# relgukxilef/GAN-Class-Transfer2

Hardware: AMD Instinct MI355X
Metric: images/sec (train step) 3x128x128 bs=64/GPU (higher is better)
Workload: dtype bf16; 1 GPU; BASELINE config 3: Trainer step, 3x128x128, bs 64/GPU, octaves 6, pixel_size 128, max_size 512, bf16 operands / fp32 accumulate, Keras Adam + WarmUp; global_batch=64, parallelism=dp1

## Files before the change

gan-class-transfer2_amd/csrc/halo_mfma.hip:

```cpp
#include "gct2_common.h"
#include <algorithm>
#include <type_traits>

namespace {

constexpr unsigned OOB = 0x80000000u;
typedef __attribute__((address_space(3))) void lds_void_t;

__device__ __forceinline__ __amdgpu_buffer_rsrc_t make_rsrc(const void* base) {
  return __builtin_amdgcn_make_buffer_rsrc(const_cast<void*>(base), 0, (int)OOB, 0x00020000);
}
__device__ __forceinline__ void dma16(__amdgpu_buffer_rsrc_t rsrc, char* lds_piece, unsigned voff) {
  __builtin_amdgcn_raw_ptr_buffer_load_lds(rsrc, (lds_void_t*)lds_piece, 16, (int)voff, 0, 0, 0);
}
__device__ __forceinline__ void dma16s(__amdgpu_buffer_rsrc_t rsrc, char* lds_piece, unsigned voff, unsigned soff) {
  __builtin_amdgcn_raw_ptr_buffer_load_lds(rsrc, (lds_void_t*)lds_piece, 16, (int)voff, (int)soff, 0, 0);
}
__device__ __forceinline__ int halo_swz(int row) { return (((row >> 1) & 1) << 2) | (((row >> 2) & 1) << 1); }
__device__ __forceinline__ int w_row(int i, int q) { return 32 * (i >> 1) + 8 * (q >> 2) + 4 * (i & 1) + (q & 3); }
__device__ __forceinline__ int w_swz(int n) { return (((n >> 3) & 1) << 1) | (((n >> 1) & 1) << 2); }

constexpr int HP = 18;
constexpr int HPIECES = 41;
constexpr int HALO_BYTES = HPIECES * 1024;
constexpr int WB_BYTES = 4 * 64 * 128;

#ifdef GCT2_STAMP
__device__ __forceinline__ unsigned long long stamp() {
  unsigned long long t;
  __builtin_amdgcn_sched_barrier(0);
  asm volatile("s_memrealtime %0\n\ts_waitcnt lgkmcnt(0)" : "=s"(t)::"memory");
  __builtin_amdgcn_sched_barrier(0);
  return t;
}
#define STAMP(k) st[k] = stamp()
#else
#define STAMP(k)
#endif
template <typename T, int EPI>
__global__ __launch_bounds__(512, 2) void halo_convT_kernel(TapGemmParams p) {
#ifdef GCT2_STAMP
  unsigned long long st[6];
  STAMP(0);
#endif
  constexpr int HEAD_CT_OFF = 2 * HALO_BYTES + 2 * WB_BYTES, HEAD_CT_BYTES = 14 * 1024;
  __shared__ __attribute__((aligned(16))) char lds_all[2 * HALO_BYTES + 2 * WB_BYTES + (EPI == EPI_HEAD ? HEAD_CT_BYTES : 0)];
  char* const halo0 = lds_all;
  char* const halo1 = lds_all + HALO_BYTES;
  char* const wb0 = lds_all + 2 * HALO_BYTES;
  char* const wb1 = lds_all + 2 * HALO_BYTES + WB_BYTES;

  GCT2_CLOCK_DECL;
  const int tid = threadIdx.x, lane = tid & 63;
  const int wave = __builtin_amdgcn_readfirstlane(tid >> 6);
  const int phase = wave >> 1, mhalf = wave & 1;
  const int ph = phase >> 1, pw = phase & 1;
  const int g = lane >> 4, q = lane & 15;
  const int Hs = p.Hs, Ws = p.Ws, K = p.K, N = p.N;
  const int tx_n = Ws >> 4, ty_n = Hs >> 4;
  int m_tile, n_tile;
  if (!xcd_tile((int)blockIdx.x, p.m_tiles, p.n_tiles, p.xcd_chunk, m_tile, n_tile)) return;
  const int tx = m_tile % tx_n, tq = m_tile / tx_n, ty = tq % ty_n, b = tq / ty_n;
  const int sh0 = ty * 16, sw0 = tx * 16, n0 = n_tile * 64;
  const __amdgpu_buffer_rsrc_t rs_x = make_rsrc(p.x), rs_w = make_rsrc(p.w);
  const int ldx2 = p.ldx * 2;

  unsigned h_voff[6];
  int h_lchunk[6];
#pragma unroll
  for (int i = 0; i < 6; i++) {
    const int pi = wave + 8 * i;
    const int row = 8 * pi + (lane >> 3);
    const int hy = row / HP, hx = row - hy * HP;
    const int lchunk = (lane & 7) ^ halo_swz(hx);
    h_lchunk[i] = lchunk;
    h_voff[i] = OOB;
    if (pi < HPIECES && row < HP * HP) {
      const int y = sh0 - 1 + hy, x = sw0 - 1 + hx;
      if ((unsigned)y < (unsigned)Hs && (unsigned)x < (unsigned)Ws) h_voff[i] = (unsigned)(((b * Hs + y) * Ws + x) * ldx2 + lchunk * 16);
    }
  }
  const int w_n = 8 * wave + (lane >> 3);
  const int w_lchunk = (lane & 7) ^ w_swz(w_n);
  const unsigned w_voff = (n0 + w_n) < N ? (unsigned)(((n0 + w_n) * K + w_lchunk * 8) * 2) : OOB;
  const unsigned NK2 = (unsigned)(N * K * 2);

  const int nk = (K + 63) / 64;
  const int nround = 4 * nk;

  auto issue_halo = [&](int kc, char* hbuf) {
    const int c0 = kc * 64;
#pragma unroll
    for (int i = 0; i < 6; i++) {
      const int pi = wave + 8 * i;
      if (pi < HPIECES)
        dma16s(rs_x, hbuf + pi * 1024, (c0 + h_lchunk[i] * 8) < K ? h_voff[i] : OOB, (unsigned)(c0 * 2));
    }
  };
  auto issue_w = [&](int round, char* wbuf) {
    const int kc = round >> 2, a = (round >> 1) & 1, c = round & 1;
    const int c0 = kc * 64;
    const unsigned voff = (c0 + w_lchunk * 8) < K ? w_voff : OOB;
#pragma unroll
    for (int i = 0; i < 4; i++) {
      const int tap16 = (1 - (i >> 1) + 2 * a) * 4 + (1 - (i & 1) + 2 * c);
      dma16s(rs_w, wbuf + i * 8192 + wave * 1024, voff, (unsigned)tap16 * NK2 + (unsigned)(c0 * 2));
    }
  };
// ... 87 lines not shown
  }
  asm volatile("s_waitcnt vmcnt(0)" ::: "memory");
  __syncthreads();
#define GCT2_LEAN_ROUND(FAST, R, IDX, HCUR, HNEXT, WCUR, WNEXT)                              \
  {                                                                                          \
    lean_round(std::integral_constant<bool, FAST>{}, (R), IDX, HCUR, HNEXT, WCUR, WNEXT);    \
    asm volatile("s_waitcnt vmcnt(0)" ::: "memory");                                         \
    __syncthreads();                                                                         \
    if (!FAST && (R) + 1 >= nround) break;                                                   \
  }
#define GCT2_LEAN_TRIP(FAST)                                                                 \
  GCT2_LEAN_ROUND(FAST, r + 0, 0, 0, HALO_BYTES, 0, WB_BYTES)                                \
  GCT2_LEAN_ROUND(FAST, r + 1, 1, 0, HALO_BYTES, WB_BYTES, 0)                                \
  GCT2_LEAN_ROUND(FAST, r + 2, 2, 0, HALO_BYTES, 0, WB_BYTES)                                \
  GCT2_LEAN_ROUND(FAST, r + 3, 3, 0, HALO_BYTES, WB_BYTES, 0)                                \
  GCT2_LEAN_ROUND(FAST, r + 4, 4, HALO_BYTES, 0, 0, WB_BYTES)                                \
  GCT2_LEAN_ROUND(FAST, r + 5, 5, HALO_BYTES, 0, WB_BYTES, 0)                                \
  GCT2_LEAN_ROUND(FAST, r + 6, 6, HALO_BYTES, 0, 0, WB_BYTES)                                \
  GCT2_LEAN_ROUND(FAST, r + 7, 7, HALO_BYTES, 0, WB_BYTES, 0)
  {
    int r = 0;
    for (; r + 8 < kfull4; r += 8) { GCT2_LEAN_TRIP(true) }
    for (; r < nround; r += 8) { GCT2_LEAN_TRIP(false) }
  }
#undef GCT2_LEAN_TRIP
#undef GCT2_LEAN_ROUND
#ifdef GCT2_STAMP
  GCT2_CLOCK_END(p.clock ? p.stamps : nullptr, 8, wave, lane);
#endif

  T* __restrict__ yout = reinterpret_cast<T*>(p.y);
  const T* __restrict__ actp = reinterpret_cast<const T*>(p.act);
  int elane = lane;
  asm volatile("" : "+v"(elane));
  const int eq = elane & 15, eg = elane >> 4;
  if constexpr (EPI == EPI_HEAD) {
    STAMP(1);
    const HeadFuse& hd = p.head;
    const int Cout = hd.Cout;
    constexpr int YP_WAVE = 64 * 128;
    constexpr int CT_OFF = HEAD_CT_OFF;
    constexpr int DT_OFF = 8 * YP_WAVE;
    constexpr int DT_WAVE = 2 * 3 * 64 * 2;
    constexpr int PC_OFF = DT_OFF + 8 * DT_WAVE;
    constexpr int LB_OFF = PC_OFF + 64;
    static_assert(LB_OFF + 256 <= HEAD_CT_OFF, "epilogue LDS map");
    auto fsw = [](int k) { return ((k >> 1) & 1) | (((k >> 3) & 1) << 1); };
    auto term_bits = head_term_bits;
    const T* __restrict__ x2 = reinterpret_cast<const T*>(hd.x2);
    const int nimg = (x2 != nullptr) ? min(hd.Cin - 64, 3) : 0;
    if (tid < 16) {
      const int c = tid >> 2, o = tid & 3;
      float v = 0.f;
      if (o < Cout) v = c < 3 ? (c < nimg ? hd.w[(64 + c) * Cout + o] : 0.f) : (hd.b ? hd.b[o] : 0.f);
      reinterpret_cast<float*>(lds_all + PC_OFF)[tid] = v;
    }
    if (tid >= 64 && tid < 128) reinterpret_cast<float*>(lds_all + LB_OFF)[tid - 64] = p.bias ? p.bias[tid - 64] : 0.f;
    __syncthreads();
    STAMP(2);
    const float gscale = (hd.loss_scale ? *hd.loss_scale : 1.f) * 2.0f / hd.count;
    float bacc[16];
    float wimg[3][3], dbd[3] = {0.f, 0.f, 0.f}, lacc = 0.f;
#pragma unroll
    for (int c = 0; c < 16; c++) bacc[c] = 0.f;
#pragma unroll
    for (int c = 0; c < 3; c++) wimg[c][0] = wimg[c][1] = wimg[c][2] = 0.f;
    f32x4_t accW[4];
#pragma unroll
    for (int f = 0; f < 4; f++) accW[f] = f32x4_t{0.f, 0.f, 0.f, 0.f};
    char* const ypark = lds_all + wave * YP_WAVE;
    char* const dtab = lds_all + DT_OFF + wave * DT_WAVE;
    const size_t pix0 = ((size_t)b * (2 * Hs) + 2 * (sh0 + mhalf * 8) + ph) * (2 * Ws) + 2 * (sw0 + eq) + pw;
    const size_t pix_step = (size_t)4 * Ws;
    auto row_pix = [&](int j) { return pix0 + (size_t)j * pix_step; };
    float tg_n[3] = {0.f, 0.f, 0.f};
    u32x2_t im_n = {0u, 0u};
    auto prefetch = [&](int j) {
      const size_t px = row_pix(j);
#pragma unroll
      for (int o = 0; o < 3; o++) tg_n[o] = o < Cout ? hd.target[px * Cout + o] : 0.f;
      if (nimg > 0) im_n = *reinterpret_cast<const u32x2_t*>(x2 + px * hd.ldx2);
    };
    prefetch(0);
#pragma unroll
    for (int j = 0; j < 8; j++) {
      int ct = CT_OFF + elane * 16;
      asm volatile("" : "+v"(ct));
      const size_t opix = row_pix(j);
      const float tg[3] = {tg_n[0], tg_n[1], tg_n[2]};
      const u32x2_t v2 = im_n;
      if (j < 7) prefetch(j + 1);
      const int krow = (j & 3) * 16 + eq;
      u32x4_t yv[2];
#pragma unroll
      for (int ip = 0; ip < 2; ip++) {
        const f32x4_t b0 = *reinterpret_cast<const f32x4_t*>(lds_all + LB_OFF + (32 * ip + 8 * eg) * 4);
        const f32x4_t b1 = *reinterpret_cast<const f32x4_t*>(lds_all + LB_OFF + (32 * ip + 8 * eg + 4) * 4);
        const f32x4_t v0 = acc[2 * ip][j] + b0, v1 = acc[2 * ip + 1][j] + b1;
        yv[ip] = u32x4_t{pack2<T>(fmaxf(v0[0], 0.f), fmaxf(v0[1], 0.f)), pack2<T>(fmaxf(v0[2], 0.f), fmaxf(v0[3], 0.f)),
                         pack2<T>(fmaxf(v1[0], 0.f), fmaxf(v1[1], 0.f)), pack2<T>(fmaxf(v1[2], 0.f), fmaxf(v1[3], 0.f))};
        *reinterpret_cast<u32x4_t*>(ypark + krow * 128 + (((2 * ip + (eg >> 1)) ^ fsw(krow)) << 5) + (eg & 1) * 16) = yv[ip];
      }
      f32x4_t accP = {0.f, 0.f, 0.f, 0.f};
#pragma unroll
      for (int t = 0; t < 3; t++)
#pragma unroll
        for (int kk = 0; kk < 2; kk++) accP = mfma16<T>(lds_read128(lds_all, ct + (t * 2 + kk) * 1024), yv[kk], accP);
      float dsc[3] = {0.f, 0.f, 0.f};
      if (eg == 0) {
        const float im[3] = {unpack_lo<T>(v2[0]), unpack_hi<T>(v2[0]), unpack_lo<T>(v2[1])};
        f32x4_t pc[4];
#pragma unroll
        for (int c = 0; c < 4; c++) pc[c] = *reinterpret_cast<const f32x4_t*>(lds_all + PC_OFF + 16 * c);
#pragma unroll
        for (int o = 0; o < 3; o++) {
          float s = accP[o];
#pragma unroll
          for (int c = 0; c < 3; c++) s = fmaf(im[c], pc[c][o], s);
          const float pr = keras_f16_point<T>(s + pc[3][o]);
          const float d = o < Cout ? pr - tg[o] : 0.f;
          if (o < Cout) {
            if (hd.pred) hd.pred[opix * Cout + o] = pr;
            lacc = fmaf(d, d, lacc);
          }
          dsc[o] = keras_f16_point<T>(d * gscale);
          dbd[o] += dsc[o];
#pragma unroll
          for (int c = 0; c < 3; c++) wimg[c][o] = fmaf(im[c], dsc[o], wimg[c][o]);
        }
      }
      u32x4_t dB[2];
#pragma unroll
      for (int t = 0; t < 2; t++) {
        const uint32_t d0 = term_bits(dsc[0], t), d1 = term_bits(dsc[1], t), d2 = term_bits(dsc[2], t);
        dB[t] = u32x4_t{d0 | (d1 << 16), d2, 0u, 0u};
        if (eg == 0) {
          uint16_t* dt = reinterpret_cast<uint16_t*>(dtab) + (t * 3) * 64 + krow;
          dt[0] = (uint16_t)d0; dt[64] = (uint16_t)d1; dt[128] = (uint16_t)d2;
        }
      }
#pragma unroll
      for (int ip = 0; ip < 2; ip++) {
        f32x4_t gq[2];
#pragma unroll
        for (int h = 0; h < 2; h++) {
          const int f = 2 * ip + h;
          const u32x4_t wh = lds_read128(lds_all, ct + (6 + f * 2) * 1024), wl = lds_read128(lds_all, ct + (7 + f * 2) * 1024);
          f32x4_t a = mfma16<T>(wh, dB[0], f32x4_t{0.f, 0.f, 0.f, 0.f});
          a = mfma16<T>(wh, dB[1], a);
          gq[h] = mfma16<T>(wl, dB[0], a);
        }
        apply_relu_bits8(relu_bits8<T>(yv[ip]), gq[0], gq[1]);
#pragma unroll
        for (int k = 0; k < 4; k++) { bacc[8 * ip + k] += gq[0][k]; bacc[8 * ip + 4 + k] += gq[1][k]; }
        const u32x4_t o = {pack2<T>(gq[0][0], gq[0][1]), pack2<T>(gq[0][2], gq[0][3]), pack2<T>(gq[1][0], gq[1][1]), pack2<T>(gq[1][2], gq[1][3])};
        *reinterpret_cast<u32x4_t*>(yout + opix * p.ldy + 32 * ip + 8 * eg) = o;
      }
      if ((j & 3) == 3) {
        asm volatile("" ::: "memory");
        const int wo = elane & 15, kg = elane >> 4;
        const int g4 = elane >> 4, q4 = (elane >> 2) & 3, pq = elane & 3;
#pragma unroll
        for (int ks = 0; ks < 2; ks++) {
          u32x4_t da[2];
#pragma unroll
          for (int t = 0; t < 2; t++) {
            da[t] = lds_read128(dtab, ((t * 3 + (wo < 3 ? wo : 0)) * 64 + 32 * ks + 8 * kg) * 2);
            if (wo >= 3) da[t] = u32x4_t{0u, 0u, 0u, 0u};
          }
          const int k0 = 32 * ks + 8 * g4 + q4;
#pragma unroll
          for (int f = 0; f < 4; f++) {
            const int o0 = k0 * 128 + ((f ^ fsw(k0)) << 5) + pq * 8;
            const s16x4_t lo = __builtin_amdgcn_ds_read_tr16_b64_v4i16((lds_s16x4_t*)(ypark + o0));
            const s16x4_t hi = __builtin_amdgcn_ds_read_tr16_b64_v4i16((lds_s16x4_t*)(ypark + o0 + 4 * 128));
            const u32x2_t l2 = __builtin_bit_cast(u32x2_t, lo), h2 = __builtin_bit_cast(u32x2_t, hi);
            const u32x4_t yb = {l2[0], l2[1], h2[0], h2[1]};
            accW[f] = mfma16<T>(da[0], yb, accW[f]);
            accW[f] = mfma16<T>(da[1], yb, accW[f]);
          }
        }
        asm volatile("" ::: "memory");
      }
    }
    STAMP(3);
    __syncthreads();
    STAMP(4);
    float* red = reinterpret_cast<float*>(lds_all);
    for (int i = tid; i < 8 * HEAD_ROW; i += 512) red[i] = 0.f;
    __syncthreads();
    float* rw = red + wave * HEAD_ROW;
    if (eg == 0) {
#pragma unroll
      for (int f = 0; f < 4; f++)
#pragma unroll
        for (int o = 0; o < 3; o++)
          if (o < Cout) rw[(16 * f + eq) * Cout + o] = accW[f][o];
    }
#pragma unroll
    for (int c = 0; c < 16; c++) {
      const float tb = row16_sum(bacc[c]);
      if (eq == 0) rw[224 + 32 * (c >> 3) + 8 * eg + (c & 7)] = tb;
    }
#pragma unroll
    for (int o = 0; o < 3; o++) {
      const float td = row16_sum(dbd[o]);
      if (elane == 0 && o < Cout) rw[216 + o] = td;
#pragma unroll
      for (int c = 0; c < 3; c++) {
        const float tw = row16_sum(wimg[c][o]);
        if (elane == 0 && o < Cout && c < nimg) rw[(64 + c) * Cout + o] = tw;
      }
    }
    {
      const float t = row16_sum(lacc);
      if (elane == 0) rw[219] = t;
    }
    __syncthreads();
    if (tid < HEAD_ROW) {
      float t = red[tid];
#pragma unroll
      for (int k = 1; k < 8; k++) t += red[k * HEAD_ROW + tid];
      hd.part[(size_t)m_tile * HEAD_ROW + tid] = t;
    }
#ifdef GCT2_STAMP
    STAMP(5);
    if (p.stamps && (tid & 63) == 0) {
      unsigned long long* o = p.stamps + ((size_t)m_tile * 8 + wave) * 8;
      for (int k = 0; k < 6; k++) o[k] = st[k];
    }
    GCT2_CLOCK_EXIT(p.clock ? p.stamps : nullptr, 8, wave, lane);
#endif
    return;
  }
  f32x4_t bsum[4];
#pragma unroll
  for (int i = 0; i < 4; i++) bsum[i] = f32x4_t{0.f, 0.f, 0.f, 0.f};
  auto out_pixel = [&](int j) {
    const int sh = sh0 + mhalf * 8 + j, sw = sw0 + eq;
    return ((size_t)b * (2 * Hs) + 2 * sh + ph) * (2 * Ws) + 2 * sw + pw;
  };
  u32x4_t mk[2] = {u32x4_t{0u, 0u, 0u, 0u}, u32x4_t{0u, 0u, 0u, 0u}};
  auto load_masks = [&](int j, u32x4_t* dst) {
    if (EPI == EPI_MASK && actp) {
      const size_t opix = out_pixel(j);
#pragma unroll
      for (int ip = 0; ip < 2; ip++) {
        const int n = n0 + 32 * ip + 8 * eg;
        if (n >= N) continue;
        if (p.bits) dst[ip][0] = p.bits[opix * p.ldbits + (n >> 3)];
        else dst[ip] = *reinterpret_cast<const u32x4_t*>(actp + opix * p.ldact + n);
      }
    }
  };
  load_masks(0, mk);
#pragma unroll
  for (int j = 0; j < 8; j++) {
    u32x4_t mkn[2] = {u32x4_t{0u, 0u, 0u, 0u}, u32x4_t{0u, 0u, 0u, 0u}};
    if (j + 1 < 8) load_masks(j + 1, mkn);
    const size_t opix = out_pixel(j);
    unsigned wbits[2] = {0u, 0u};
#pragma unroll
    for (int ip = 0; ip < 2; ip++) {
      const int n = n0 + 32 * ip + 8 * eg;
      if (n >= N) continue;
      f32x4_t v0 = acc[2 * ip][j], v1 = acc[2 * ip + 1][j];
      if (EPI == EPI_BIAS_ACT) {
        if (p.bias) {
          v0 += *reinterpret_cast<const f32x4_t*>(p.bias + n);
          v1 += *reinterpret_cast<const f32x4_t*>(p.bias + n + 4);
        }
        if (p.relu) {
#pragma unroll
          for (int r = 0; r < 4; r++) { v0[r] = fmaxf(v0[r], 0.f); v1[r] = fmaxf(v1[r], 0.f); }
        }
      } else {
        if (actp && p.bits) apply_relu_bits8(mk[ip][0], v0, v1);
        else if (actp) {
          const u32x4_t a4 = mk[ip];
#pragma unroll
          for (int h = 0; h < 2; h++) {
            if (!(unpack_lo<T>(a4[h]) > 0.f)) v0[2 * h] = 0.f;
            if (!(unpack_hi<T>(a4[h]) > 0.f)) v0[2 * h + 1] = 0.f;
            if (!(unpack_lo<T>(a4[2 + h]) > 0.f)) v1[2 * h] = 0.f;
            if (!(unpack_hi<T>(a4[2 + h]) > 0.f)) v1[2 * h + 1] = 0.f;
          }
        }
        bsum[2 * ip] += v0;
        bsum[2 * ip + 1] += v1;
        if (p.accumulate) {
          const u32x4_t o4 = *reinterpret_cast<const u32x4_t*>(yout + opix * p.ldy + n);
#pragma unroll
          for (int h = 0; h < 2; h++) {
            v0[2 * h] += unpack_lo<T>(o4[h]); v0[2 * h + 1] += unpack_hi<T>(o4[h]);
            v1[2 * h] += unpack_lo<T>(o4[2 + h]); v1[2 * h + 1] += unpack_hi<T>(o4[2 + h]);
          }
        }
      }
      const u32x4_t o = {pack2<T>(v0[0], v0[1]), pack2<T>(v0[2], v0[3]), pack2<T>(v1[0], v1[1]), pack2<T>(v1[2], v1[3])};
      *reinterpret_cast<u32x4_t*>(yout + opix * p.ldy + n) = o;
      if (EPI == EPI_BIAS_ACT && p.bits && !p.bits_words) p.bits[opix * p.ldbits + (n >> 3)] = (unsigned char)relu_bits8<T>(o);
      if (EPI == EPI_BIAS_ACT && p.bits_words) wbits[ip] = relu_bits8<T>(o) << (8 * eg);
    }
    if (EPI == EPI_BIAS_ACT && p.bits_words) {
#pragma unroll
      for (int ip = 0; ip < 2; ip++) {
        const unsigned wd = rows4_or(wbits[ip]);
        if (eg == 0 && n0 + 32 * ip < N) *reinterpret_cast<unsigned*>(p.bits + opix * p.ldbits + ((n0 + 32 * ip) >> 3)) = wd;
      }
    }
    mk[0] = mkn[0]; mk[1] = mkn[1];
    __builtin_amdgcn_sched_barrier(0);
  }
  if (EPI == EPI_MASK && (p.db || p.db2)) {
    float* red = reinterpret_cast<float*>(wb0);
#pragma unroll
    for (int i = 0; i < 4; i++) {
#pragma unroll
      for (int r = 0; r < 4; r++) {
        float t = bsum[i][r];
        t = row16_sum(t);
        const int c = 32 * (i >> 1) + 8 * eg + 4 * (i & 1) + r;
        if (eq == 0) {
          if (p.dbws) red[wave * 64 + c] = t;
          else if (n0 + c < N) {
            float* qd = (n0 + c) < p.db_split ? (p.db ? p.db + n0 + c : nullptr) : (p.db2 ? p.db2 + (n0 + c - p.db_split) : nullptr);
            if (qd) atomicAdd(qd, t);
          }
        }
      }
    }
    if (p.dbws) {
      __syncthreads();
      if (tid < 64 && n0 + tid < N) {
        float t = red[tid];
#pragma unroll
        for (int k = 1; k < 8; k++) t += red[k * 64 + tid];
        p.dbws[(size_t)m_tile * N + n0 + tid] = t;
      }
    }
  }
#ifdef GCT2_STAMP
  GCT2_CLOCK_EXIT(p.clock ? p.stamps : nullptr, 8, wave, lane);
#endif
}

}

bool halo_convT_wanted(const gct2_ctx& c, int epi, const TapGemmParams& p) {
  const int g_halo_mode = c.halo_mode;
  if (g_halo_mode == 1) return false;
  if ((p.Hs & 15) || (p.Ws & 15)) return false;
  if ((uintptr_t)p.y % 16 || p.ldy % 8 || (p.act && ((uintptr_t)p.act % 16 || p.ldact % 8))) return false;
  if (g_halo_mode == 2) return true;
  const int tiles = p.B * (p.Hs >> 4) * (p.Ws >> 4) * ((p.N + 63) / 64);
  return p.N <= 256 && tiles >= 256;
}

bool halo_head_supported(const gct2_ctx& c, int dtype, const TapGemmParams& p) {
  if (dtype != GCT2_BF16 && dtype != GCT2_F16) return false;
  if (p.N != 64 || (p.Hs & 15) || (p.Ws & 15) || p.K % 8 || p.ldx % 8) return false;
  if ((uintptr_t)p.y % 16 || p.ldy % 8 || (uintptr_t)p.x % 16 || (uintptr_t)p.w % 16) return false;
  const size_t src_bytes = (size_t)p.B * p.Hs * p.Ws * p.ldx * 2, lane_max = 7 * 16 + 16, scalar_max = (size_t)p.K * 2;
  const size_t w_bytes = (size_t)16 * p.K * p.N * 2;
  if (src_bytes + lane_max + scalar_max >= 0x7ff00000u || w_bytes >= 0x7ff00000u) return false;
  const size_t rows = (size_t)p.B * (p.Hs >> 4) * (p.Ws >> 4);
  return c.ws && c.ws_bytes >= rows * HEAD_ROW * sizeof(float);
}
int halo_head(gct2_ctx& c, int dtype, TapGemmParams p, float* dw, float* db, float* loss, float* db_up, int accumulate,
              hipStream_t s) {
  p.m_tiles = p.B * (p.Hs >> 4) * (p.Ws >> 4);
  p.n_tiles = 1;
  p.xcd_chunk = (p.m_tiles + 7) / 8;
  p.ksplit = 1;
// ... 56 lines not shown
```

gan-class-transfer2_amd/csrc/tapgemm_mfma.hip:

```cpp
#include "gct2_common.h"
#include <algorithm>


namespace {

constexpr int BK = 64;
constexpr unsigned OOB = 0x80000000u;
#define VMCNT_ONLY(n) ((((n) & 0xF) | 0x70 | 0xF00 | ((((n) >> 4) & 3) << 14)))
typedef __attribute__((address_space(3))) void lds_void_t;

__device__ __forceinline__ __amdgpu_buffer_rsrc_t make_rsrc(const void* base) {
  return __builtin_amdgcn_make_buffer_rsrc(const_cast<void*>(base), 0, (int)OOB, 0x00020000);
}
__device__ __forceinline__ void dma16(__amdgpu_buffer_rsrc_t rsrc, char* lds_piece, unsigned voff) {
  __builtin_amdgcn_raw_ptr_buffer_load_lds(rsrc, (lds_void_t*)lds_piece, 16, (int)voff, 0, 0, 0);
}
__device__ __forceinline__ void dma16s(__amdgpu_buffer_rsrc_t rsrc, char* lds_piece, unsigned voff, unsigned soff) {
  __builtin_amdgcn_raw_ptr_buffer_load_lds(rsrc, (lds_void_t*)lds_piece, 16, (int)voff, (int)soff, 0, 0);
}

__device__ __forceinline__ float* db_target(const TapGemmParams& p, int n) {
  return n < p.db_split ? (p.db ? p.db + n : nullptr) : (p.db2 ? p.db2 + (n - p.db_split) : nullptr);
}
__device__ __forceinline__ bool db_adds(const TapGemmParams& p, int n) { return (p.db_acc >> (n < p.db_split ? 0 : 1)) & 1; }

#ifdef GCT2_STAMP
__device__ __forceinline__ unsigned long long tg_stamp() {
  unsigned long long t;
  __builtin_amdgcn_sched_barrier(0);
  asm volatile("s_memrealtime %0\n\ts_waitcnt lgkmcnt(0)" : "=s"(t)::"memory");
  __builtin_amdgcn_sched_barrier(0);
  return t;
}
#define TG_STAMP(k) st[k] = tg_stamp()
#else
#define TG_STAMP(k)
#endif
template <typename T, int FORM, int BM, int BN, int EPI, int NBUF>
__global__ __launch_bounds__((BM / 64) * (BN / 64) * 64, NBUF == 1 ? 4 : 2) void tapgemm_kernel(TapGemmParams p) {
  constexpr int WM = 64;
  constexpr int NWV = (BM / WM) * (BN / 64);
  constexpr int MF = WM / 16;
  static_assert(NBUF == 1 || NBUF == 2, "one or two LDS buffers");
  static_assert(NWV == 4 || NWV == 8, "4 or 8 waves");
  constexpr bool S1 = (FORM == FORM_S1 || FORM == FORM_S1T);
  constexpr bool WT = (FORM == FORM_CONV || FORM == FORM_S1);
  static_assert(!WT || BN % 128 == 0, "T images are 128 columns wide");
  constexpr int WAVES_N = BN / 64;
  constexpr int BKS = BK;
  constexpr int NA = BM / 8 / NWV;
  constexpr int NW = (WT ? 16 * (BN / 128) : BN / 8) / NWV;
  constexpr int A_BYTES = BM * 128;
  constexpr int W_BYTES = WT ? 64 * 256 * (BN / 128) : BN * 128;
  constexpr int NTAPS = (FORM == FORM_CONV) ? 16 : 4;

  __shared__ __attribute__((aligned(16))) char lds0[A_BYTES + W_BYTES];
  __shared__ __attribute__((aligned(16))) char lds1[NBUF >= 2 ? A_BYTES + W_BYTES : 16];

#ifdef GCT2_STAMP
  unsigned long long st[5];
  unsigned long long* stamp_out = p.stamps;
  TG_STAMP(0);
#endif
  GCT2_CLOCK_DECL;
  const int tid = threadIdx.x, lane = tid & 63;
  const int wave = __builtin_amdgcn_readfirstlane(tid >> 6);
  const int wn = wave % WAVES_N, wm = wave / WAVES_N;
  const int Hs = p.Hs, Ws = p.Ws, K = p.K, N = p.N;
  const int M = p.B * Hs * Ws;
  constexpr int PH = (FORM == FORM_CONVT) ? 4 : 1;
  const int inner = p.n_tiles * PH, per_slice = 8 * p.xcd_chunk * inner;
  int kslice, m_tile, in;
  if (p.wstat) {
    const int xcd = (int)blockIdx.x & 7, j = (int)blockIdx.x >> 3;
    const int slice = (j / p.m_tiles) * 8 + xcd;
    if (slice >= inner * p.ksplit) return;
    m_tile = j % p.m_tiles;
    kslice = slice / inner;
    in = slice - kslice * inner;
  } else {
    kslice = (int)blockIdx.x / per_slice;
    if (!xcd_tile((int)blockIdx.x - kslice * per_slice, p.m_tiles, inner, p.xcd_chunk, m_tile, in)) return;
  }
  const int phase = in % PH, n_tile = in / PH;
  const int m0 = m_tile * BM, n0 = n_tile * BN;
  const int ph = phase >> 1, pw = phase & 1;
  const int Hsrc = (FORM == FORM_CONV) ? 2 * Hs : Hs, Wsrc = (FORM == FORM_CONV) ? 2 * Ws : Ws;
  const __amdgpu_buffer_rsrc_t rs_x = make_rsrc(p.x), rs_w = make_rsrc(p.w);
  const int ldx2 = p.ldx * 2;
// ... 138 lines not shown
    const char* w_img = a_img + A_BYTES;
#pragma unroll
    for (int kk = 0; kk < 2; kk++) {
      u32x4_t wf[4], af[MF];
#pragma unroll
      for (int i = 0; i < 4; i++)
        wf[i] = WT ? timg_frag(w_img + (wn >> 1) * (64 * 256), (wn & 1) * 64 + i * 16, kk, lane)
                                    : nimg_frag(w_img, wn * 64 + i * 16, kk, lane);
#pragma unroll
      for (int j = 0; j < MF; j++) af[j] = nimg_frag(a_img, wm * WM + j * 16, kk, lane);
#pragma unroll
      for (int i = 0; i < 4; i++)
#pragma unroll
        for (int j = 0; j < MF; j++) acc[i][j] = mfma16<T>(wf[i], af[j], acc[i][j]);
    }
  };
  const bool live = p.ksplit > 0;
  TG_STAMP(1);
  GCT2_CLOCK_BEGIN;
  if constexpr (NBUF == 1) {
    for (int it = it_lo; it < it_hi; it++) {
      issue(it, lds0);
      asm volatile("s_waitcnt vmcnt(0)" ::: "memory");
      __syncthreads();
      if (live) compute(lds0);
      __syncthreads();
    }
  } else if constexpr (NBUF == 2) {
    if (it_lo < it_hi) issue(it_lo, lds0);
    asm volatile("s_waitcnt vmcnt(0)" ::: "memory");
    __syncthreads();
    for (int it = it_lo; it < it_hi; it += 2) {
      if (it + 1 < it_hi) issue(it + 1, lds1);
      if (live) compute(lds0);
      asm volatile("s_waitcnt vmcnt(0)" ::: "memory");
      __syncthreads();
      if (it + 1 >= it_hi) break;
      if (it + 2 < it_hi) issue(it + 2, lds0);
      if (live) compute(lds1);
      asm volatile("s_waitcnt vmcnt(0)" ::: "memory");
      __syncthreads();
    }
  }

#ifdef GCT2_STAMP
  GCT2_CLOCK_END(p.clock ? p.stamps : nullptr, NWV, wave, lane);
#endif
  TG_STAMP(2);
  T* __restrict__ yout = reinterpret_cast<T*>(p.y);
  const T* __restrict__ actp = reinterpret_cast<const T*>(p.act);
  int elane = lane;
  asm volatile("" : "+v"(elane));
  f32x4_t bsum[4];
#pragma unroll
  for (int i = 0; i < 4; i++) bsum[i] = f32x4_t{0.f, 0.f, 0.f, 0.f};
  const bool wide = p.wide && p.ksplit == 1;
  if (wide) {
    const int eg = elane >> 4;
    const int nlane = wn * 64 + 16 * (eg & 1) + 4 * (eg & ~1);
    auto out_pixel = [&](int j, size_t& opix) -> bool {
      const int m = m0 + wm * WM + j * 16 + (elane & 15);
      if (m >= M) return false;
      if (FORM != FORM_CONVT) opix = (size_t)m;
      else {
        int sw, sh, b;
        decode_pixel(m, Hs, Ws, p.hs_shift, p.ws_shift, sw, sh, b);
        opix = ((size_t)b * (2 * Hs) + 2 * sh + ph) * (2 * Ws) + 2 * sw + pw;
      }
      return true;
    };
    u32x4_t mk[2] = {u32x4_t{0u, 0u, 0u, 0u}, u32x4_t{0u, 0u, 0u, 0u}};
    auto load_masks = [&](int j, u32x4_t* dst) {
      size_t opix;
      if (EPI == EPI_MASK && actp && out_pixel(j, opix)) {
#pragma unroll
        for (int ip = 0; ip < 2; ip++) {
          const int n = n0 + nlane + 32 * ip;
          if (n >= N) continue;
          if (p.bits) dst[ip][0] = p.bits[opix * p.ldbits + (n >> 3)];
          else dst[ip] = *reinterpret_cast<const u32x4_t*>(actp + opix * p.ldact + n);
        }
      }
    };
    load_masks(0, mk);
#pragma unroll
    for (int j = 0; j < MF; j++) {
      u32x4_t mkn[2] = {u32x4_t{0u, 0u, 0u, 0u}, u32x4_t{0u, 0u, 0u, 0u}};
      if (j + 1 < MF) load_masks(j + 1, mkn);
      f32x4_t v0[2], v1[2];
#pragma unroll
      for (int ip = 0; ip < 2; ip++) {
#pragma unroll
        for (int r = 0; r < 4; r++) {
          float xa = acc[2 * ip][j][r], xb = acc[2 * ip + 1][j][r];
          asm volatile("v_permlane16_swap_b32 %0, %1" : "+v"(xa), "+v"(xb));
          v0[ip][r] = xa;
          v1[ip][r] = xb;
        }
      }
      size_t opix;
      const bool row_ok = out_pixel(j, opix);
      unsigned wbits[2] = {0u, 0u};
#pragma unroll
      for (int ip = 0; ip < 2; ip++) {
        const int n = n0 + nlane + 32 * ip;
        if (!row_ok || n >= N) continue;
        f32x4_t a = v0[ip], c = v1[ip];
        if (EPI == EPI_BIAS_ACT) {
          if (p.bias) {
            a += *reinterpret_cast<const f32x4_t*>(p.bias + n);
            c += *reinterpret_cast<const f32x4_t*>(p.bias + n + 4);
          }
          if (p.relu) {
#pragma unroll
            for (int r = 0; r < 4; r++) { a[r] = fmaxf(a[r], 0.f); c[r] = fmaxf(c[r], 0.f); }
          }
        } else {
          if (actp && p.bits) apply_relu_bits8(mk[ip][0], a, c);
          else if (actp) {
            const u32x4_t a4 = mk[ip];
#pragma unroll
            for (int h = 0; h < 2; h++) {
              if (!(unpack_lo<T>(a4[h]) > 0.f)) a[2 * h] = 0.f;
              if (!(unpack_hi<T>(a4[h]) > 0.f)) a[2 * h + 1] = 0.f;
              if (!(unpack_lo<T>(a4[2 + h]) > 0.f)) c[2 * h] = 0.f;
              if (!(unpack_hi<T>(a4[2 + h]) > 0.f)) c[2 * h + 1] = 0.f;
            }
          }
          bsum[2 * ip] += a;
          bsum[2 * ip + 1] += c;
          if (p.accumulate) {
            const u32x4_t o4 = *reinterpret_cast<const u32x4_t*>(yout + opix * p.ldy + n);
#pragma unroll
            for (int h = 0; h < 2; h++) {
              a[2 * h] += unpack_lo<T>(o4[h]); a[2 * h + 1] += unpack_hi<T>(o4[h]);
              c[2 * h] += unpack_lo<T>(o4[2 + h]); c[2 * h + 1] += unpack_hi<T>(o4[2 + h]);
            }
          }
        }
        const u32x4_t o = {pack2<T>(a[0], a[1]), pack2<T>(a[2], a[3]), pack2<T>(c[0], c[1]), pack2<T>(c[2], c[3])};
        *reinterpret_cast<u32x4_t*>(yout + opix * p.ldy + n) = o;
        if (EPI == EPI_BIAS_ACT && p.bits && !p.bits_words) p.bits[opix * p.ldbits + (n >> 3)] = (unsigned char)relu_bits8<T>(o);
        if (EPI == EPI_BIAS_ACT && p.bits_words) wbits[ip] = relu_bits8<T>(o) << (((n >> 3) & 3) * 8);
      }
      if (EPI == EPI_BIAS_ACT && p.bits_words) {
#pragma unroll
        for (int ip = 0; ip < 2; ip++) {
          const unsigned wd = rows4_or(wbits[ip]);
          const int n32 = n0 + wn * 64 + 32 * ip;
          if (eg == 0 && row_ok && n32 < N) *reinterpret_cast<unsigned*>(p.bits + opix * p.ldbits + (n32 >> 3)) = wd;
        }
      }
      mk[0] = mkn[0]; mk[1] = mkn[1];
      __builtin_amdgcn_sched_barrier(0);
    }
  } else {
#pragma unroll
  for (int j = 0; j < MF; j++) {
    const int m = m0 + wm * WM + j * 16 + (elane & 15);
    if (m >= M) continue;
    size_t opix;
    if (FORM != FORM_CONVT) opix = (size_t)m;
    else {
      int sw, sh, b;
      decode_pixel(m, Hs, Ws, p.hs_shift, p.ws_shift, sw, sh, b);
      opix = ((size_t)b * (2 * Hs) + 2 * sh + ph) * (2 * Ws) + 2 * sw + pw;
    }
#pragma unroll
    for (int i = 0; i < 4; i++) {
      const int n = n0 + wn * 64 + i * 16 + 4 * (elane >> 4);
      if (n >= N) continue;
      f32x4_t v = acc[i][j];
      if (p.ksplit > 1) {
        const size_t npix = (size_t)M * (FORM == FORM_CONVT ? 4 : 1);
        *reinterpret_cast<f32x4_t*>(p.ws + ((size_t)kslice * npix + opix) * N + n) = v;
        continue;
      }
      if (EPI == EPI_BIAS_ACT) {
        if (p.bias) {
          const f32x4_t bv = *reinterpret_cast<const f32x4_t*>(p.bias + n);
          v += bv;
        }
        if (p.relu) {
#pragma unroll
          for (int r = 0; r < 4; r++) v[r] = fmaxf(v[r], 0.f);
        }
      } else {
        if (actp) {
          const u32x2_t a2 = *reinterpret_cast<const u32x2_t*>(actp + opix * p.ldact + n);
          if (!(unpack_lo<T>(a2[0]) > 0.f)) v[0] = 0.f;
          if (!(unpack_hi<T>(a2[0]) > 0.f)) v[1] = 0.f;
          if (!(unpack_lo<T>(a2[1]) > 0.f)) v[2] = 0.f;
          if (!(unpack_hi<T>(a2[1]) > 0.f)) v[3] = 0.f;
        }
        bsum[i] += v;
        if (p.accumulate) {
          const u32x2_t o2 = *reinterpret_cast<const u32x2_t*>(yout + opix * p.ldy + n);
          v[0] += unpack_lo<T>(o2[0]); v[1] += unpack_hi<T>(o2[0]);
          v[2] += unpack_lo<T>(o2[1]); v[3] += unpack_hi<T>(o2[1]);
        }
      }
      u32x2_t o = {pack2<T>(v[0], v[1]), pack2<T>(v[2], v[3])};
      *reinterpret_cast<u32x2_t*>(yout + opix * p.ldy + n) = o;
    }
    __builtin_amdgcn_sched_barrier(0);
  }
  }
  TG_STAMP(3);
#ifdef GCT2_STAMP
  if (stamp_out && lane == 0) {
    TG_STAMP(4);
    unsigned long long* o = stamp_out + ((size_t)blockIdx.x * NWV + wave) * 8;
    for (int k = 0; k < 5; k++) o[k] = st[k];
  }
#endif
  if (EPI == EPI_MASK && (p.db || p.db2) && p.ksplit == 1) {
    float* red = reinterpret_cast<float*>(lds0);
    constexpr int WAVES_M = NWV / WAVES_N;
#pragma unroll
    for (int i = 0; i < 4; i++) {
#pragma unroll
      for (int r = 0; r < 4; r++) {
        float t = bsum[i][r];
        t = row16_sum(t);
        const int eg2 = elane >> 4;
        const int c = wide ? wn * 64 + 32 * (i >> 1) + 16 * (eg2 & 1) + 4 * (eg2 & ~1) + 4 * (i & 1) + r
                           : wn * 64 + i * 16 + 4 * eg2 + r;
        if ((elane & 15) == 0) {
          if (p.dbws) red[wm * BN + c] = t;
          else if (n0 + c < N) {
            float* q = db_target(p, n0 + c);
            if (q) atomicAdd(q, t);
          }
        }
      }
    }
    if (p.dbws) {
      __syncthreads();
      if (tid < BN && n0 + tid < N) {
        float t = red[tid];
#pragma unroll
        for (int k = 1; k < WAVES_M; k++) t += red[k * BN + tid];
        p.dbws[(size_t)(m_tile * PH + phase) * N + n0 + tid] = t;
      }
    }
  }
#ifdef GCT2_STAMP
  GCT2_CLOCK_EXIT(p.clock ? p.stamps : nullptr, NWV, wave, lane);
#endif
}

__global__ __launch_bounds__(1024) void dbpart_reduce_kernel(const float* __restrict__ part, int rows, TapGemmParams p) {
  const int N = p.N;
  const int tid = threadIdx.x, cq = tid & 7, rl = tid >> 3;
  const int n = blockIdx.x * 32 + cq * 4;
  f32x4_t acc = {0.f, 0.f, 0.f, 0.f};
  if (n < N)
    for (int r = rl; r < rows; r += 128) acc += *reinterpret_cast<const f32x4_t*>(part + (size_t)r * N + n);
#pragma unroll
  for (int k = 0; k < 4; k++) {
    float t = acc[k];
    t += __shfl_xor(t, 8, 64); t += __shfl_xor(t, 16, 64); t += __shfl_xor(t, 32, 64);
    acc[k] = t;
  }
  __shared__ f32x4_t red[16][8];
  if ((tid & 63) < 8) red[tid >> 6][cq] = acc;
  __syncthreads();
  if (tid < 8 && n < N) {
    f32x4_t t = red[0][tid];
#pragma unroll
    for (int k = 1; k < 16; k++) t += red[k][tid];
#pragma unroll
    for (int r = 0; r < 4; r++) {
      float* q = db_target(p, n + r);
      if (q) *q = db_adds(p, n + r) ? *q + t[r] : t[r];
    }
  }
}

struct DbJobs { int njobs, phase; int blk0[17]; gct2_ctx::DbJob j[16]; };
__global__ __launch_bounds__(1024) void dbpart_reduce_multi_kernel(const DbJobs J) {
  int k = 0;
  while (k + 1 < J.njobs && (int)blockIdx.x >= J.blk0[k + 1]) k++;
  const gct2_ctx::DbJob job = J.j[k];
  const int N = job.N, rows = job.rows;
  const float* __restrict__ part = job.part;
  const int tid = threadIdx.x, cq = tid & 7, rl = tid >> 3;
  const int n = ((int)blockIdx.x - J.blk0[k]) * 32 + cq * 4;
// ... 276 lines not shown
```

Measured before the change: 26140 images/sec.

## Software-pipeline halo head rows and prefetch accumulate-read outputs in epilogues

In the halo convT kernel, the bias/relu/pack and projection MFMAs for row j+1 now run ahead of row j's loss and weight-gradient work, and parking into LDS is deferred until after row j's reads. In both the halo and tapgemm epilogues, the previous output values needed for accumulate mode are loaded one or more rows ahead so their global-load latency overlaps other work. The tapgemm non-mask epilogue also moves the ksplit branch out of the inner loop. This raises register pressure with double-buffered yv/accP and prefetched outputs, which could reduce occupancy under the 512x2 launch bounds.

```diff
diff --git a/gan-class-transfer2_amd/csrc/halo_mfma.hip b/gan-class-transfer2_amd/csrc/halo_mfma.hip
--- a/gan-class-transfer2_amd/csrc/halo_mfma.hip
+++ b/gan-class-transfer2_amd/csrc/halo_mfma.hip
@@ -24,6 +24,9 @@
 constexpr int HPIECES = 41;
 constexpr int HALO_BYTES = HPIECES * 1024;
 constexpr int WB_BYTES = 4 * 64 * 128;
+#ifndef GCT2_HALO_ACC_AHEAD
+#define GCT2_HALO_ACC_AHEAD 1
+#endif
 
 #ifdef GCT2_STAMP
 __device__ __forceinline__ unsigned long long stamp() {
@@ -277,8 +280,36 @@
       if (nimg > 0) im_n = *reinterpret_cast<const u32x2_t*>(x2 + px * hd.ldx2);
     };
     prefetch(0);
+    u32x4_t yvS[2][2];
+    f32x4_t accPS[2];
+    auto front_row = [&](int j, u32x4_t* yv, f32x4_t& accP) __attribute__((always_inline)) {
+      int ct = CT_OFF + elane * 16;
+      asm volatile("" : "+v"(ct));
+#pragma unroll
+      for (int ip = 0; ip < 2; ip++) {
+        const f32x4_t b0 = *reinterpret_cast<const f32x4_t*>(lds_all + LB_OFF + (32 * ip + 8 * eg) * 4);
+        const f32x4_t b1 = *reinterpret_cast<const f32x4_t*>(lds_all + LB_OFF + (32 * ip + 8 * eg + 4) * 4);
+        const f32x4_t v0 = acc[2 * ip][j] + b0, v1 = acc[2 * ip + 1][j] + b1;
+        yv[ip] = u32x4_t{pack2<T>(fmaxf(v0[0], 0.f), fmaxf(v0[1], 0.f)), pack2<T>(fmaxf(v0[2], 0.f), fmaxf(v0[3], 0.f)),
+                         pack2<T>(fmaxf(v1[0], 0.f), fmaxf(v1[1], 0.f)), pack2<T>(fmaxf(v1[2], 0.f), fmaxf(v1[3], 0.f))};
+      }
+      accP = f32x4_t{0.f, 0.f, 0.f, 0.f};
+#pragma unroll
+      for (int t = 0; t < 3; t++)
+#pragma unroll
+        for (int kk = 0; kk < 2; kk++) accP = mfma16<T>(lds_read128(lds_all, ct + (t * 2 + kk) * 1024), yv[kk], accP);
+    };
+    auto park_row = [&](int j, const u32x4_t* yv) __attribute__((always_inline)) {
+      const int krow = (j & 3) * 16 + eq;
+#pragma unroll
+      for (int ip = 0; ip < 2; ip++)
+        *reinterpret_cast<u32x4_t*>(ypark + krow * 128 + (((2 * ip + (eg >> 1)) ^ fsw(krow)) << 5) + (eg & 1) * 16) = yv[ip];
+    };
+    front_row(0, yvS[0], accPS[0]);
+    park_row(0, yvS[0]);
 #pragma unroll
     for (int j = 0; j < 8; j++) {
+      if (j < 7) front_row(j + 1, yvS[(j + 1) & 1], accPS[(j + 1) & 1]);
       int ct = CT_OFF + elane * 16;
       asm volatile("" : "+v"(ct));
       const size_t opix = row_pix(j);
@@ -286,21 +317,8 @@
       const u32x2_t v2 = im_n;
       if (j < 7) prefetch(j + 1);
       const int krow = (j & 3) * 16 + eq;
-      u32x4_t yv[2];
-#pragma unroll
-      for (int ip = 0; ip < 2; ip++) {
-        const f32x4_t b0 = *reinterpret_cast<const f32x4_t*>(lds_all + LB_OFF + (32 * ip + 8 * eg) * 4);
-        const f32x4_t b1 = *reinterpret_cast<const f32x4_t*>(lds_all + LB_OFF + (32 * ip + 8 * eg + 4) * 4);
-        const f32x4_t v0 = acc[2 * ip][j] + b0, v1 = acc[2 * ip + 1][j] + b1;
-        yv[ip] = u32x4_t{pack2<T>(fmaxf(v0[0], 0.f), fmaxf(v0[1], 0.f)), pack2<T>(fmaxf(v0[2], 0.f), fmaxf(v0[3], 0.f)),
-                         pack2<T>(fmaxf(v1[0], 0.f), fmaxf(v1[1], 0.f)), pack2<T>(fmaxf(v1[2], 0.f), fmaxf(v1[3], 0.f))};
-        *reinterpret_cast<u32x4_t*>(ypark + krow * 128 + (((2 * ip + (eg >> 1)) ^ fsw(krow)) << 5) + (eg & 1) * 16) = yv[ip];
-      }
-      f32x4_t accP = {0.f, 0.f, 0.f, 0.f};
-#pragma unroll
-      for (int t = 0; t < 3; t++)
-#pragma unroll
-        for (int kk = 0; kk < 2; kk++) accP = mfma16<T>(lds_read128(lds_all, ct + (t * 2 + kk) * 1024), yv[kk], accP);
+      const u32x4_t yv[2] = {yvS[j & 1][0], yvS[j & 1][1]};
+      const f32x4_t accP = accPS[j & 1];
       float dsc[3] = {0.f, 0.f, 0.f};
       if (eg == 0) {
         const float im[3] = {unpack_lo<T>(v2[0]), unpack_hi<T>(v2[0]), unpack_lo<T>(v2[1])};
@@ -377,6 +395,7 @@
         }
         asm volatile("" ::: "memory");
       }
+      if (j < 7) park_row(j + 1, yvS[(j + 1) & 1]);
     }
     STAMP(3);
     __syncthreads();
@@ -448,11 +467,29 @@
       }
     }
   };
+  constexpr int ACC_AHEAD = GCT2_HALO_ACC_AHEAD;
+  u32x4_t ov[ACC_AHEAD][2];
+  auto load_prev = [&](int j, u32x4_t* dst) {
+    dst[0] = dst[1] = u32x4_t{0u, 0u, 0u, 0u};
+    if (EPI == EPI_MASK && p.accumulate) {
+      const size_t opix = out_pixel(j);
+#pragma unroll
+      for (int ip = 0; ip < 2; ip++) {
+        const int n = n0 + 32 * ip + 8 * eg;
+        if (n >= N) continue;
+        dst[ip] = *reinterpret_cast<const u32x4_t*>(yout + opix * p.ldy + n);
+      }
+    }
+  };
   load_masks(0, mk);
+#pragma unroll
+  for (int d = 0; d < ACC_AHEAD; d++) load_prev(d, ov[d]);
 #pragma unroll
   for (int j = 0; j < 8; j++) {
     u32x4_t mkn[2] = {u32x4_t{0u, 0u, 0u, 0u}, u32x4_t{0u, 0u, 0u, 0u}};
     if (j + 1 < 8) load_masks(j + 1, mkn);
+    const u32x4_t oj[2] = {ov[j % ACC_AHEAD][0], ov[j % ACC_AHEAD][1]};
+    if (j + ACC_AHEAD < 8) load_prev(j + ACC_AHEAD, ov[j % ACC_AHEAD]);
     const size_t opix = out_pixel(j);
     unsigned wbits[2] = {0u, 0u};
 #pragma unroll
@@ -484,7 +521,7 @@
         bsum[2 * ip] += v0;
         bsum[2 * ip + 1] += v1;
         if (p.accumulate) {
-          const u32x4_t o4 = *reinterpret_cast<const u32x4_t*>(yout + opix * p.ldy + n);
+          const u32x4_t o4 = oj[ip];
 #pragma unroll
           for (int h = 0; h < 2; h++) {
             v0[2 * h] += unpack_lo<T>(o4[h]); v0[2 * h + 1] += unpack_hi<T>(o4[h]);
diff --git a/gan-class-transfer2_amd/csrc/tapgemm_mfma.hip b/gan-class-transfer2_amd/csrc/tapgemm_mfma.hip
--- a/gan-class-transfer2_amd/csrc/tapgemm_mfma.hip
+++ b/gan-class-transfer2_amd/csrc/tapgemm_mfma.hip
@@ -5,6 +5,10 @@
 namespace {
 
 constexpr int BK = 64;
+#ifndef GCT2_TAP_ACC_AHEAD
+#define GCT2_TAP_ACC_AHEAD 1
+#endif
+constexpr int ACC_AHEAD = GCT2_TAP_ACC_AHEAD;
 constexpr unsigned OOB = 0x80000000u;
 #define VMCNT_ONLY(n) ((((n) & 0xF) | 0x70 | 0xF00 | ((((n) >> 4) & 3) << 14)))
 typedef __attribute__((address_space(3))) void lds_void_t;
@@ -309,11 +313,29 @@
         }
       }
     };
+    constexpr int AH = NBUF == 1 ? 0 : (ACC_AHEAD < MF ? ACC_AHEAD : MF), AHN = AH > 0 ? AH : 1;
+    u32x4_t ov[AHN][2] = {};
+    auto load_prev = [&](int j, u32x4_t* dst) {
+      dst[0] = dst[1] = u32x4_t{0u, 0u, 0u, 0u};
+      size_t opix;
+      if (EPI == EPI_MASK && p.accumulate && out_pixel(j, opix)) {
+#pragma unroll
+        for (int ip = 0; ip < 2; ip++) {
+          const int n = n0 + nlane + 32 * ip;
+          if (n >= N) continue;
+          dst[ip] = *reinterpret_cast<const u32x4_t*>(yout + opix * p.ldy + n);
+        }
+      }
+    };
     load_masks(0, mk);
+#pragma unroll
+    for (int d = 0; d < AH; d++) load_prev(d, ov[d]);
 #pragma unroll
     for (int j = 0; j < MF; j++) {
       u32x4_t mkn[2] = {u32x4_t{0u, 0u, 0u, 0u}, u32x4_t{0u, 0u, 0u, 0u}};
       if (j + 1 < MF) load_masks(j + 1, mkn);
+      const u32x4_t oj[2] = {ov[j % AHN][0], ov[j % AHN][1]};
+      if (AH > 0 && j + AH < MF) load_prev(j + AH, ov[j % AHN]);
       f32x4_t v0[2], v1[2];
 #pragma unroll
       for (int ip = 0; ip < 2; ip++) {
@@ -357,7 +379,8 @@
           bsum[2 * ip] += a;
           bsum[2 * ip + 1] += c;
           if (p.accumulate) {
-            const u32x4_t o4 = *reinterpret_cast<const u32x4_t*>(yout + opix * p.ldy + n);
+            u32x4_t o4 = oj[ip];
+            if constexpr (AH == 0) o4 = *reinterpret_cast<const u32x4_t*>(yout + opix * p.ldy + n);
 #pragma unroll
             for (int h = 0; h < 2; h++) {
               a[2 * h] += unpack_lo<T>(o4[h]); a[2 * h + 1] += unpack_hi<T>(o4[h]);
@@ -382,27 +405,59 @@
       __builtin_amdgcn_sched_barrier(0);
     }
   } else {
-#pragma unroll
-  for (int j = 0; j < MF; j++) {
+  auto out_pixel = [&](int j, size_t& opix) -> bool {
     const int m = m0 + wm * WM + j * 16 + (elane & 15);
-    if (m >= M) continue;
-    size_t opix;
+    if (m >= M) return false;
     if (FORM != FORM_CONVT) opix = (size_t)m;
     else {
       int sw, sh, b;
       decode_pixel(m, Hs, Ws, p.hs_shift, p.ws_shift, sw, sh, b);
       opix = ((size_t)b * (2 * Hs) + 2 * sh + ph) * (2 * Ws) + 2 * sw + pw;
     }
+    return true;
+  };
+  if (p.ksplit > 1) {
+    const size_t npix = (size_t)M * (FORM == FORM_CONVT ? 4 : 1);
+#pragma unroll
+    for (int j = 0; j < MF; j++) {
+      size_t opix;
+      if (!out_pixel(j, opix)) continue;
+#pragma unroll
+      for (int i = 0; i < 4; i++) {
+        const int n = n0 + wn * 64 + i * 16 + 4 * (elane >> 4);
+        if (n >= N) continue;
+        *reinterpret_cast<f32x4_t*>(p.ws + ((size_t)kslice * npix + opix) * N + n) = acc[i][j];
+      }
+      __builtin_amdgcn_sched_barrier(0);
+    }
+  } else {
+  constexpr int AH = NBUF == 1 ? 0 : (ACC_AHEAD < MF ? ACC_AHEAD : MF), AHN = AH > 0 ? AH : 1;
+  u32x2_t ov[AHN][4] = {};
+  auto load_prev = [&](int j, u32x2_t* dst) {
+    dst[0] = dst[1] = dst[2] = dst[3] = u32x2_t{0u, 0u};
+    size_t opix;
+    if (EPI == EPI_MASK && p.accumulate && out_pixel(j, opix)) {
+#pragma unroll
+      for (int i = 0; i < 4; i++) {
+        const int n = n0 + wn * 64 + i * 16 + 4 * (elane >> 4);
+        if (n >= N) continue;
+        dst[i] = *reinterpret_cast<const u32x2_t*>(yout + opix * p.ldy + n);
+      }
+    }
+  };
+#pragma unroll
+  for (int d = 0; d < AH; d++) load_prev(d, ov[d]);
+#pragma unroll
+  for (int j = 0; j < MF; j++) {
+    size_t opix;
+    if (!out_pixel(j, opix)) continue;
+    const u32x2_t oj[4] = {ov[j % AHN][0], ov[j % AHN][1], ov[j % AHN][2], ov[j % AHN][3]};
+    if (AH > 0 && j + AH < MF) load_prev(j + AH, ov[j % AHN]);
 #pragma unroll
     for (int i = 0; i < 4; i++) {
       const int n = n0 + wn * 64 + i * 16 + 4 * (elane >> 4);
       if (n >= N) continue;
       f32x4_t v = acc[i][j];
-      if (p.ksplit > 1) {
-        const size_t npix = (size_t)M * (FORM == FORM_CONVT ? 4 : 1);
-        *reinterpret_cast<f32x4_t*>(p.ws + ((size_t)kslice * npix + opix) * N + n) = v;
-        continue;
-      }
       if (EPI == EPI_BIAS_ACT) {
         if (p.bias) {
           const f32x4_t bv = *reinterpret_cast<const f32x4_t*>(p.bias + n);
@@ -422,7 +477,8 @@
         }
         bsum[i] += v;
         if (p.accumulate) {
-          const u32x2_t o2 = *reinterpret_cast<const u32x2_t*>(yout + opix * p.ldy + n);
+          u32x2_t o2 = oj[i];
+          if constexpr (AH == 0) o2 = *reinterpret_cast<const u32x2_t*>(yout + opix * p.ldy + n);
           v[0] += unpack_lo<T>(o2[0]); v[1] += unpack_hi<T>(o2[0]);
           v[2] += unpack_lo<T>(o2[1]); v[3] += unpack_hi<T>(o2[1]);
         }
@@ -431,6 +487,7 @@
       *reinterpret_cast<u32x2_t*>(yout + opix * p.ldy + n) = o;
     }
     __builtin_amdgcn_sched_barrier(0);
+  }
   }
   }
   TG_STAMP(3);
```

Measured after the change: 26340 images/sec, median of 6. About the same (+0.8%).
